# X1X1010/XequiNet

Measured on AMD Instinct MI355X. Metric: edges/sec + achieved HBM GB/s, energy+force inference, QM9-shape batch, higher is better.
Workload: dtype f32

## Files before the change

include/xeq.h:

```cpp
#ifndef XEQ_H
#define XEQ_H
#include <stdint.h>

#ifdef __cplusplus
extern "C" {
#endif

enum { XEQ_F32 = 0, XEQ_F64 = 1 };
enum { XEQ_RBF_BESSEL = 0, XEQ_RBF_GAUSSIAN = 1, XEQ_RBF_EXPBERN = 2, XEQ_RBF_EXPNORM = 3 };
enum { XEQ_CUTOFF_COSINE = 0, XEQ_CUTOFF_POLYNOMIAL = 1 };
enum {
  XEQ_OK = 0,
  XEQ_ERR_INVALID_ARGUMENT = 1,
  XEQ_ERR_LAUNCH = 2,
  XEQ_ERR_UNSUPPORTED = 3
};

int xeq_version(void);
const char* xeq_last_error(void);
int64_t xeq_launch_count(void);
int64_t xeq_launch_names(int64_t first, char* buf, int64_t cap);


int xeq_csr_rowptr(const int64_t* keys, int64_t n_keys, int64_t n_rows, int32_t* rowptr, void* stream);
// ... 317 lines not shown
int64_t xeq_rowptr_from_degrees_max(void);

int xeq_node_block_supported(int dtype, int node_dim, const int32_t mul[3]);
int xeq_node_block_auto(int64_t n);
int64_t xeq_small_rows_limit(void);
int xeq_node_block_set_waves(int waves);
int64_t xeq_node_block_rows(int64_t n);
int64_t xeq_node_block_fwd_tiles(int with_tail);
int xeq_node_block_pack_fwd(const float* w3, const float* uv0, const float* uv1, const float* uv2, const float* dot, const float* w4,
                            const float* w1_next, const float* w2_next, void* out, void* stream);
int xeq_node_block_fwd(int64_t n, const float* s, const float* x, const float* ln_w, const float* ln_b, const float* eq_w, const float* eq_b,
                       const float* b_uv, const float* b3, const float* b4, double eps, const void* packed, float* p_scratch, float* uv_bt, float* stats,
                       float* pre, float* a, float* ip, float* s_out, float* x_out, const float* ln_w_next, const float* ln_b_next,
                       const float* eq_w_next, const float* eq_b_next, const float* b1_next, const float* b2_next, float* stats_next,
                       float* xhat_next, float* pre_next, float* h_next, void* stream);
int64_t xeq_node_block_bwd_tiles(int with_tail, int with_gx);
int xeq_node_block_pack_bwd(const float* w3, const float* uv0, const float* uv1, const float* uv2, const float* dot, const float* w4,
                            const float* w1_next, const float* w2_next, int with_gx, void* out, void* stream);
int xeq_node_block_bwd(int64_t n, const float* g_h, const float* g_xhat_next, const float* g_s_in, const float* g_x_in, const float* s_out,
                       const float* x_out, const float* stats_next, const float* pre_next, const float* ln_w_next, const float* eq_w_next,
                       const float* uv_bt, const float* a, const float* ip, const float* pre, const float* s, const float* x,
                       const float* stats, const float* ln_w, const float* eq_w, double eps, const void* packed, float* gxo, float* gp,
                       float* gv, float* gw, float* g_s, float* g_x, void* stream);
int xeq_node_block_linear_test(const float* x, int64_t n, const float* w, int n_ot, int form, void* packed_scratch, float* y, void* stream);

#ifdef __cplusplus
}
#endif
#endif
```

xequinet_amd/csrc/xeq_nodeblock.hip:

```cpp
#include <stdlib.h>
#include <atomic>

#include <vector>

#include "xeq_common.h"

namespace xeq {
namespace nb {

typedef float tile_t __attribute__((ext_vector_type(8)));
typedef float f32x4 __attribute__((ext_vector_type(4)));
typedef float f32x8 __attribute__((ext_vector_type(8)));
typedef __bf16 bf16x8 __attribute__((ext_vector_type(8)));

constexpr int F = 128, M0 = 128, M1 = 64, M2 = 32, C = M0 + M1 + M2, D = M0 + 3 * M1 + 5 * M2;
constexpr int HM = F + 2 * C;
constexpr int AU = C + 2 * F;
constexpr int WAVE_ROWS = 16;
constexpr int ROWS_WG = 64;
constexpr int MAX_WAVES = 8;
constexpr int TILE_U4 = 192;
#ifndef XEQ_NB_STAGE
#define XEQ_NB_STAGE 4
#endif
// ... 541 lines not shown

struct FwdArgs {
  int64_t n;
  const float *s, *x;
  const float *lnw, *lnb, *eqw, *eqb;
  const float* b_uv;
  const float *b3, *b4;
  float eps;
  const uint4* wp;
  int n_tiles;
  float* p;
  float *uv, *stats, *pre, *a, *ip;
  float *s_out, *x_out;
  const float *lnw2, *lnb2, *eqw2, *eqb2, *b1n, *b2n;
  float *stats2, *xhat2, *pre2, *h2;
};

template <bool TAIL>
__global__ void __launch_bounds__(64 * MAX_WAVES, 1) k_node_block_fwd(FwdArgs a) {
  extern __shared__ uint4 ring[];
  const int lane = threadIdx.x & 63, wave = __builtin_amdgcn_readfirstlane(threadIdx.x >> 6);
  const int n = lane & 15, h = lane >> 4;
  const int n_waves = (int)(blockDim.x >> 6);
  const int64_t node = ((int64_t)blockIdx.x * n_waves + wave) * WAVE_ROWS + n;
  const bool ok = node < a.n;
  const int64_t row = ok ? node : a.n - 1;
  const int64_t N = a.n;
  NB_STAMP(0);
  NB_RSTAMP(17);
  WStream w;
  w.init(a.wp, ring, a.n_tiles, lane, wave & 3);
  const Park pk{ring + RING_BYTES / 16 + wave * PARK_U4 + lane};
  NB_STAMP(1);
// ... 208 lines not shown
      }
      st_xm<5>(xor_ + M0 + 3 * M1, h, X, ok);
    }
  }
  NB_STAMP(8);
  tile_t IP[4] = {zero16(), zero16(), zero16(), zero16()};
  {
    tile_t pt = ld_nat(pw, 0, lane);
    for (int t = 0; t < 7; ++t) {
      const tile_t cur = pt;
      if (t + 1 < 7) pt = ld_nat(pw, t + 1, lane);
      accum_tile<4>(w, IP, cur);
    }
  }
  tile_t SN[4];
  float* __restrict__ sor = a.s_out + row * F;
#pragma unroll
  for (int c = 0; c < 4; ++c) {
    const tile_t bsv = ld_par(a.b4, C + 32 * c, h), bss = ld_par(a.b4, C + F + 32 * c, h), S = ld_tile(srow, 32 * c, h);
    NB_SAVE(st_nat(ipw, c, lane, IP[c]));
    tile_t asv = zero16(), ass = zero16();
    out_pair_p<4>(w, asv, ass, pk);
    asv += bsv;
    ass += bss;
    NB_SAVE(st_nat(aw, 7 + c, lane, asv));
    NB_SAVE(st_nat(aw, 11 + c, lane, ass));
#pragma unroll
    for (int r = 0; r < 8; ++r) SN[c][r] = (S[r] + asv[r] * IP[c][r]) + ass[r];
    st_tile(sor, 32 * c, h, SN[c], ok);
  }
  NB_STAMP(9);
  if (!TAIL) return;

  const float mean_n = row_sum((sum16(SN[0]) + sum16(SN[1])) + (sum16(SN[2]) + sum16(SN[3]))) * (1.f / F);
  const float var_n = row_sum((sumsq16(SN[0], mean_n) + sumsq16(SN[1], mean_n)) + (sumsq16(SN[2], mean_n) + sumsq16(SN[3], mean_n))) * (1.f / F);
  const float rstd_n = 1.f / sqrtf(var_n + 1e-5f);
  const float mean0_n = row_sum(s0) * (1.f / M0);
  tile_t XN0[4];
#pragma unroll
  for (int t = 0; t < 4; ++t) XN0[t] = ld_tile(xor_, 32 * t, h);
  tile_t HN[4] = {zero16(), zero16(), zero16(), zero16()};
#pragma unroll
  for (int t = 0; t < 4; ++t) {
    const tile_t wv = ld_par(a.lnw2, 32 * t, h), bv = ld_par(a.lnb2, 32 * t, h);
    tile_t sh;
#pragma unroll
// ... 58 lines not shown
      }
    }
  }
  NB_STAMP(13);
  NB_RSTAMP(18);
#ifdef XEQ_NB_STAMPS
  if (lane == 0 && blockIdx.x < 1024) {
    g_nb_stamps[((int)blockIdx.x * 4 + wave) * NB_STAMPS + 14] = w.t_commit;
    g_nb_stamps[((int)blockIdx.x * 4 + wave) * NB_STAMPS + 15] = w.t_barrier;
    unsigned hw_, xcc_;
    asm volatile("s_getreg_b32 %0, hwreg(HW_REG_HW_ID)" : "=s"(hw_));
    asm volatile("s_getreg_b32 %0, hwreg(HW_REG_XCC_ID)" : "=s"(xcc_));
    g_nb_stamps[((int)blockIdx.x * 4 + wave) * NB_STAMPS + 16] = ((unsigned long long)xcc_ << 32) | hw_;
  }
#endif
}

enum { B_W2N = 0, B_W1N = 1, B_W4 = 2, B_W3 = 3, B_DOT = 4, B_UV0 = 5, B_UV1 = 6, B_UV2 = 7 };
static void program_bwd(bool tail, bool gx, std::vector<Seg>& p) {
  p.clear();
  if (tail) {
    p.push_back({B_W2N, 0, 4, 1, 0, HM / 32, 1, 0});
    p.push_back({B_W1N, 0, 4, 1, 0, 4, 1, 1});
  }
  if (gx) p.push_back({B_W4, 0, 4, 1, 0, 7, 1, 0});
  p.push_back({B_W4, 0, 4, 1, 7, 8, 1, 0});
  p.push_back({B_W3, 0, 4, 1, 0, 4, 1, 1});
  p.push_back({B_W3, 4, 7, 1, 0, 4, 1, 1});
  p.push_back({B_DOT, 0, 7, 1, 0, 4, 1, 1});
  for (int c = 0; c < 4; ++c) p.push_back({B_UV0, 0, 4, 1, c, 2, M0 / 32, 0});
// ... 454 lines not shown
    for (int m = 0; m < 5; ++m) {
      GW[m] = ld_nat(gww, x_tile(2, m, 0), lane);
      if (GX) R[m] = ld_nat(gxow, x_tile(2, m, 0), lane);
    }
#pragma unroll
    for (int m = 0; m < 5; ++m)
#pragma unroll
      for (int r = 0; r < 8; ++r) X[m][r] = (rr * GW[m][r] - coef * X[m][r]) + (GX ? R[m][r] : 0.f);
    st_xm<5>(gxr + M0 + 3 * M1, h, X, ok);
  }
}

static hipError_t raise_lds() {
  static hipError_t err = [] {
    const void* fns[] = {reinterpret_cast<const void*>(&k_node_block_fwd<true>), reinterpret_cast<const void*>(&k_node_block_fwd<false>),
                         reinterpret_cast<const void*>(&k_node_block_bwd<true, true>), reinterpret_cast<const void*>(&k_node_block_bwd<false, true>),
                         reinterpret_cast<const void*>(&k_node_block_bwd<false, false>)};
    hipError_t e = hipSuccess;
    for (const void* f : fns) {
      const hipError_t r = hipFuncSetAttribute(f, hipFuncAttributeMaxDynamicSharedMemorySize, lds_bytes(MAX_WAVES));
      if (r != hipSuccess) e = r;
    }
    return e;
  }();
  return err;
}

static std::atomic<int> g_waves_override{0};
static int waves_for(int64_t n) {
  const char* v = getenv("XEQ_NODE_BLOCK_WAVES");
// ... 77 lines not shown
                "xeq_node_block_fwd: null buffer");
  XEQ_CHECK_ARG(!tail || (x_out && ln_w_next && ln_b_next && eq_w_next && eq_b_next && b1_next && b2_next && stats_next && xhat_next && pre_next),
                "xeq_node_block_fwd: null buffer (next block)");
  FwdArgs fa;
  fa.n = n; fa.s = s; fa.x = x; fa.lnw = ln_w; fa.lnb = ln_b; fa.eqw = eq_w; fa.eqb = eq_b; fa.b_uv = b_uv; fa.b3 = b3; fa.b4 = b4;
  fa.eps = (float)eps; fa.wp = (const uint4*)packed; fa.n_tiles = (int)xeq_node_block_fwd_tiles(tail);
  fa.p = p_scratch; fa.uv = uv_bt; fa.stats = stats; fa.pre = pre; fa.a = a; fa.ip = ip; fa.s_out = s_out; fa.x_out = x_out;
  fa.lnw2 = ln_w_next; fa.lnb2 = ln_b_next; fa.eqw2 = eq_w_next; fa.eqb2 = eq_b_next; fa.b1n = b1_next; fa.b2n = b2_next;
  fa.stats2 = stats_next; fa.xhat2 = xhat_next; fa.pre2 = pre_next; fa.h2 = h_next;
  const int nw = waves_for(n);
  const dim3 grid((unsigned)((n + nw * WAVE_ROWS - 1) / (nw * WAVE_ROWS)));
  XEQ_CHECK_ARG(raise_lds() == hipSuccess, "xeq_node_block_fwd: cannot raise the dynamic LDS limit");
  if (tail) hipLaunchKernelGGL(k_node_block_fwd<true>, grid, dim3(64 * nw), lds_bytes(nw), (hipStream_t)stream, fa);
  else hipLaunchKernelGGL(k_node_block_fwd<false>, grid, dim3(64 * nw), lds_bytes(nw), (hipStream_t)stream, fa);
  XEQ_CHECK_LAUNCH("xeq_node_block_fwd");
  return XEQ_OK;
}

int64_t xeq_node_block_bwd_tiles(int with_tail, int with_gx) {
  std::vector<Seg> p;
  program_bwd(with_tail != 0, with_gx != 0 || with_tail != 0, p);
  return padded_tiles(seg_tiles(p));
}

int xeq_node_block_pack_bwd(const float* w3, const float* uv0, const float* uv1, const float* uv2, const float* dot, const float* w4,
                            const float* w1n, const float* w2n, int with_gx, void* out, void* stream) {
  XEQ_CHECK_ARG(w3 && uv0 && uv1 && uv2 && dot && w4 && out && ((w1n == nullptr) == (w2n == nullptr)), "xeq_node_block_pack_bwd: null buffer");
  const bool tail = w1n != nullptr;
  std::vector<Seg> p;
  program_bwd(tail, tail || with_gx != 0, p);
// ... 55 lines not shown
```

xequinet_amd/csrc/xeq_torch.cpp:

```cpp
#include <ATen/ATen.h>
#include <c10/hip/HIPStream.h>
#include <hip/hip_runtime_api.h>
#include <torch/csrc/autograd/custom_function.h>
#include <torch/library.h>

#include <cmath>
#include <cstdlib>
#include <mutex>
#include <optional>
#include <unordered_map>
#include <vector>

#include "../../include/xeq.h"

namespace {

using at::Tensor;
using torch::autograd::AutogradContext;
using torch::autograd::variable_list;

#define XCALL(...)                                                                                  \
  do {                                                                                              \
    const int st_ = (__VA_ARGS__);                                                                  \
    TORCH_CHECK(st_ == 0, "xequinet_amd: ", #__VA_ARGS__, " failed (", st_, "): ", xeq_last_error()); \
// ... 615 lines not shown
                            g.fwd.dbasis.defined() ? g.fwd.dbasis.data_ptr() : nullptr, st));
  } else {
    const int w = xeq_edge_basis_width(hy.B);
    g.sb_basis = at::empty({E, w}, fopt);
    g.sb_dbasis = at::empty({E, w}, fopt);
    XCALL(xeq_edge_basis(dt, vec.data_ptr(), E, hy.rbf_kind, hy.cutoff_kind, hy.B, hy.cutoff, p0.data_ptr(), OP(p1),
                         g.sb_basis.data_ptr(), g.sb_dbasis.data_ptr(), st));
  }

  auto wq_w = [&](const Tensor* q) {
    const Tensor* pk = wq_weight_pack(q[4], q[5], hy.B, F, mul);
    TORCH_CHECK(pk != nullptr, "xeq::xpainn_eval: rbf_lin weights cannot be packed for the wq kernels");
    return pk;
  };
  const bool nb_ok = dt == XEQ_F32 && hy.layer_norm && xeq_node_block_supported(XEQ_F32, F, mul) && xeq_node_block_auto(N);
  for (int b = 0; b < hy.blocks; ++b) {
    const Tensor* q = &prm[P_BLOCK0 + P_PER_BLOCK * b];
    {
      MsgSaved& m = msv[b];
      if (b > 0 && !m.h.defined()) {
        m.s = s;
        m.x = x;
        NormOut no = norm_fwd(hy, s, x, q[6], q[7], q[8], q[9], Tensor(), 0);
        m.stats = no.stats;
        m.xhat = no.xhat;
        mlp_fwd(no.shat, q[0], q[1], q[2], q[3], m.pre, m.h);
      }
      Tensor s_out = at::empty_like(s), x_out = at::empty_like(x);
      m.impl = impl;
      if (impl == 0) {
// ... 17 lines not shown
      u.s = s;
      u.x = x;
      const bool last_blk = b == hy.blocks - 1;
      if (nb_ok) {
        const Tensor* qn = last_blk ? nullptr : &prm[P_BLOCK0 + P_PER_BLOCK * (b + 1)];
        const NbPacks* pk = nb_packs(q, qn, !last_blk);
        auto fp = [](const Tensor& t) { return t.defined() ? (const float*)t.data_ptr() : nullptr; };
        auto fpm = [](Tensor& t) { return t.defined() ? (float*)t.data_ptr() : nullptr; };
        const int64_t NR = xeq_node_block_rows(N);
        u.uv = at::empty({2 * NR * D}, fopt);
        u.stats = at::empty({N, 4}, fopt);
        u.pre = at::empty({NR, F}, fopt);
        u.a = at::empty({NR, C + 2 * F}, fopt);
        u.ip = at::empty({NR, F}, fopt);
        Tensor p_scr = at::empty({NR, C}, fopt);
        Tensor s_out = at::empty_like(s), x_out = last_blk ? Tensor() : at::empty_like(x);
        MsgSaved* mn = last_blk ? nullptr : &msv[b + 1];
        if (mn) {
          mn->stats = at::empty({N, 4}, fopt);
          mn->xhat = at::empty({N * D}, fopt);
          mn->pre = at::empty({NR, F}, fopt);
          mn->h = at::empty({N, H}, fopt);
        }
        XCALL(xeq_node_block_fwd(N, fp(s), fp(x), fp(q[19]), fp(q[20]), fp(q[21]), fp(q[22]), fp(pk->bias_uv), fp(q[16]), fp(q[18]),
                                 hy.inv_eps, pk->fwd.data_ptr(), fpm(p_scr), fpm(u.uv), fpm(u.stats), fpm(u.pre), fpm(u.a), fpm(u.ip),
                                 fpm(s_out), fpm(x_out), qn ? fp(qn[6]) : nullptr, qn ? fp(qn[7]) : nullptr, qn ? fp(qn[8]) : nullptr,
                                 qn ? fp(qn[9]) : nullptr, qn ? fp(qn[1]) : nullptr, qn ? fp(qn[3]) : nullptr,
                                 mn ? fpm(mn->stats) : nullptr, mn ? fpm(mn->xhat) : nullptr, mn ? fpm(mn->pre) : nullptr,
                                 mn ? fpm(mn->h) : nullptr, st));
        s = s_out;
// ... 23 lines not shown
          const Tensor& W = q[10 + xb[k].l];
          if (xb[k].l == 0 && q[13].numel() > 0) at::addmm_out(ub[k].view, q[13], xb[k].view, W);
          else at::mm_out(ub[k].view, xb[k].view, W);
        }
        XCALL(xeq_uv_reduce_fwd(dt, u.uv.data_ptr(), N, mul, hy.inv_eps, cat.data_ptr(), F + C, F, p.data_ptr(), st));
      }
      mlp_and_linear_fwd(cat, q[15], q[16], q[17], q[18], p, q[14], u.pre, u.a, u.ip);
      const bool last = b == hy.blocks - 1;
      Tensor s_out = at::empty_like(s), x_out = last ? Tensor() : at::empty_like(x);
      XCALL(xeq_update_out_fwd(dt, s.data_ptr(), x.data_ptr(), u.uv.data_ptr(), u.a.data_ptr(), u.ip.data_ptr(), N, F, mul,
                               s_out.data_ptr(), last ? nullptr : x_out.data_ptr(), st));
      s = s_out;
      x = x_out;
    }
  }
  const Tensor* t = &prm[P_BLOCK0 + P_PER_BLOCK * hy.blocks];
  const LinPack* head_pk = dt == XEQ_F32 && t[0].size(0) % 4 == 0 && t[2].size(0) == 1 ? lin_pack(t[0], t[1]) : nullptr;
  const bool head_native = head_pk != nullptr && head_pk->bwd.defined();
  Tensor pre_o, atomic, jac;
  const bool head_fused = head_native && s.stride(1) == 1 && s.stride(0) % 4 == 0 && t[1].defined() && t[1].numel() > 0 &&
                          xeq_head_supported(XEQ_F32, F, (int)t[0].size(0));
  if (head_fused) {
    atomic = at::empty({N}, fopt);
    if (compute_forces || compute_virial) jac = at::empty({N, (int64_t)F}, fopt);
    XCALL(xeq_head_fwd(s.data_ptr(), s.stride(0), N, F, (int)t[0].size(0), head_pk->fwd.data_ptr(), head_pk->bwd.data_ptr(), t[2].data_ptr(),
                       t[3].data_ptr(), atomic.data_ptr(), jac.defined() ? jac.data_ptr() : nullptr, st));
  } else if (head_native) {
    const Tensor hidden = linear_fwd(s, t[0], t[1], 1, nullptr, &pre_o);
    atomic = at::empty({N}, fopt);
    XCALL(xeq_head_dot(hidden.data_ptr(), N, (int)t[0].size(0), t[2].data_ptr(), t[3].data_ptr(), atomic.data_ptr(), st));
  } else {
    pre_o = at::addmm(t[1], s, t[0].t());
    atomic = at::addmm(t[3], at::silu(pre_o), t[2].t()).reshape({-1});
  }
  Tensor energy = at::empty({G}, fopt);
  XCALL(xeq_segment_sum(dt, atomic.data_ptr(), (const int64_t*)ptr64.data_ptr(), G, 1, energy.data_ptr(), st));

// ... 339 lines not shown
```

xequinet_amd/lib.py:

```python
from __future__ import annotations

import ctypes
import os
from ctypes import c_char_p, c_double, c_int, c_int32, c_int64, c_void_p
from typing import Optional

import torch

_HERE = os.path.dirname(os.path.abspath(__file__))
LIB_PATH = os.environ.get("XEQ_LIB_PATH") or os.path.join(_HERE, "libxeq_hip.so")

XEQ_F32, XEQ_F64 = 0, 1
COPY_MANY_MAX = 16
SB_ACCUM_VEC = 16
XHAT_HIGHER_L_ZERO = 2
SB_Y0_ZERO = 8
SB_Q_ACCUMULATE = 16
SB_NO_GY = 32
WQ_MIRROR_WALK = 4
WQ_PACKED_WEIGHTS = 64
WQ_MAX_PART_SETS = 8
RBF_KINDS = {"bessel": 0, "gaussian": 1, "expbern": 2, "expnorm": 3}
CUTOFF_KINDS = {"cosine": 0, "polynomial": 1}

# ... 134 lines not shown
    "xeq_mlp2_fwd": [_P, c_int64, c_int64, c_int, _P, _P, c_int, _P, _P, c_int64, _P],
    "xeq_mlp2_bwd": [_P, c_int64, c_int64, c_int, _P, _P, _P, c_int, _P, c_int64, _P],
    "xeq_mlp2_and_linear": [c_int, _P, c_int64, c_int64, c_int, _P, _P, c_int, _P, _P, c_int64, _P, c_int64, c_int, _P, c_int, _P, c_int64, _P],
    "xeq_pack_epoch": [],
    "xeq_pack_epoch_bump": [],
    "xeq_rowptr_guard": [_P, c_int64, c_int64, _P, _P, _P],
    "xeq_node_block_supported": [c_int, c_int, _I3],
    "xeq_node_block_fwd_tiles": [c_int],
    "xeq_node_block_rows": [c_int64],
    "xeq_node_block_auto": [c_int64],
    "xeq_small_rows_limit": [],
    "xeq_node_block_set_waves": [c_int],
    "xeq_node_block_pack_fwd": [_P, _P, _P, _P, _P, _P, _P, _P, _P, _P],
    "xeq_node_block_fwd": [c_int64, _P, _P, _P, _P, _P, _P, _P, _P, _P, c_double, _P, _P, _P, _P, _P, _P, _P, _P, _P, _P, _P, _P, _P, _P, _P,
                           _P, _P, _P, _P, _P],
    "xeq_node_block_linear_test": [_P, c_int64, _P, c_int, c_int, _P, _P, _P],
    "xeq_node_block_bwd_tiles": [c_int, c_int],
    "xeq_node_block_pack_bwd": [_P, _P, _P, _P, _P, _P, _P, _P, c_int, _P, _P],
    "xeq_node_block_bwd": [c_int64, _P, _P, _P, _P, _P, _P, _P, _P, _P, _P, _P, _P, _P, _P, _P, _P, _P, _P, _P, c_double, _P, _P, _P, _P, _P,
                           _P, _P, _P],
}
_RET_I64 = {"xeq_launch_count", "xeq_launch_names", "xeq_message_wq_packed_weight_floats", "xeq_rowptr_from_degrees_max", "xeq_csr_by_key_workspace", "xeq_message_wq_pcap", "xeq_message_wq_plan_workspace", "xeq_message_wq_win_ints",
            "xeq_message_wq_parts_floats", "xeq_mlp_packed_floats", "xeq_exclusive_scan_i32_workspace", "xeq_node_block_fwd_tiles", "xeq_node_block_bwd_tiles", "xeq_node_block_rows", "xeq_pack_epoch", "xeq_tensor_product_wgrad_chunks", "xeq_small_rows_limit"}
EXPORTS = ["xeq_version", "xeq_last_error", *_PROTOS]

_lib: Optional[ctypes.CDLL] = None


def load() -> ctypes.CDLL:
    global _lib
# ... 81 lines not shown
```

xequinet_amd/nn/fused.py:

```python
from __future__ import annotations

import math
from typing import Tuple

import torch
import torch.nn.functional as F_
from torch.autograd import Function
from torch.autograd.function import once_differentiable

from .. import lib, ops
from ..lib import call, dtype_code, mul3, ptr, stream

def _bt_blocks(buf: torch.Tensor, n: int, mul, width: int):
    out = []
    base = 0
    for l, m in enumerate(mul):
        d = 2 * l + 1
        if m > 0:
            out.append((l, m, buf[n * base * width : n * (base + d * m) * width].view(n * d, width * m)))
        base += d * m
    return out


def _norm_fwd(s, x, norm, o3norm, node_dim, mul, shat_out=None, ld=None):
# ... 316 lines not shown
    @staticmethod
    @once_differentiable
    def backward(ctx, g_atomic, g_total):
        if not ctx.saved_tensors or (g_atomic is None and g_total is None):
            return None, None, None, None
        jac, batch = ctx.saved_tensors
        n, F = jac.shape
        if g_atomic is not None and g_atomic.stride(0) not in (0, 1):
            g_atomic = g_atomic.contiguous()
        if g_total is not None and g_total.stride(0) not in (0, 1):
            g_total = g_total.contiguous()
        g_s = torch.empty_like(jac)
        call("xeq_head_bwd", ptr(jac), n, F, ptr(g_atomic), 0 if g_atomic is None else g_atomic.stride(0), ptr(g_total),
             0 if g_total is None else g_total.stride(0), ptr(batch), ptr(g_s), stream())
        return g_s, None, None, None


class EmbeddingLinear(Function):

    @staticmethod
    def forward(ctx, z32, table, lin, weight, bias):
        out = _linear(table, _linear_pack(lin, weight, bias, False), weight.shape[1], weight.shape[0], bias is not None, row_index=z32)[0]
        ctx.save_for_backward(z32, table)
        ctx.has_bias = bias is not None
        return out

    @staticmethod
    @once_differentiable
    def backward(ctx, g):
        z32, table = ctx.saved_tensors
# ... 289 lines not shown
```

xequinet_amd/nn/model.py:

```python
from __future__ import annotations

from typing import Dict, Iterable, List, Optional, Union

import torch
import torch.nn as nn

from . import training
from .basic import compute_edge_data, compute_properties
from .output import resolve_output
from .xpainn import XEmbedding, XPainnMessage, XPainnUpdate

_E3NN_ONLY = (".rsh_conv.", ".tp.", ".scalar_mul.", ".sph_harm.", ".output_mask", "._", ".invariant.tp", ".equidot.tp")


class BaseModel(nn.Module):
    cutoff_radius: float

    def __init__(self) -> None:
        super().__init__()
        self.mods = nn.ModuleDict()
        self.extra_properties = []
        self.native_training = True

    def forward(
# ... 76 lines not shown
            )
        if action_blocks > 0:
            self.mods["embedding"]._next_message = [self.mods["message_0"]]
        for i in range(action_blocks - 1):
            self.mods[f"update_{i}"]._next_message = [self.mods[f"message_{i + 1}"]]
        if output_modes is None:
            output_modes = ["energy"]
        elif isinstance(output_modes, str) or not isinstance(output_modes, Iterable):
            output_modes = [output_modes]
        for mode in output_modes:
            output = resolve_output(mode, **kwargs)
            self.mods[f"output_{mode}"] = output
            self.extra_properties.extend(output.extra_properties)
        if action_blocks > 0 and all(not getattr(self.mods[f"output_{m}"], "reads_equivariant", False) for m in output_modes):
            self.mods[f"update_{action_blocks - 1}"].equivariant_output_unused = True


def resolve_model(model_name: str, **kwargs) -> BaseModel:
    models_factory = {"xpainn": XPaiNN}
    if model_name.lower() not in models_factory:
        raise NotImplementedError(f"Unsupported model {model_name}")
    return models_factory[model_name.lower()](**kwargs)


def load_model(ckpt_file: str, device: Optional[torch.device] = None):
    from ..data import NeighborTransform

    class ModelWithTransform:
        def __init__(self, model, transform, device):
            self.model = model
# ... 17 lines not shown
```

xequinet_amd/nn/nodeblock.py:

```python
from __future__ import annotations

from typing import Optional

import torch

from .. import lib
from ..lib import call, mul3, ptr, stream

TILE_BYTES = 3072
pack_epoch = lib.pack_epoch


def supported(update, message=None) -> bool:
    from .fused import _packed_uv

    if not isinstance(update.update_mlp[1], torch.nn.SiLU) or isinstance(update.norm, torch.nn.Identity):
        return False
    w = update.update_mlp[0].weight
    if w.dtype != torch.float32 or not w.is_cuda:
        return False
    if not lib.load().xeq_node_block_supported(lib.XEQ_F32, update.node_dim, mul3(update.node_irreps.mul3())):
        return False
    if update.update_mlp[0].bias is None or update.update_mlp[2].bias is None or update.dot_lin.bias is not None:
        return False
# ... 67 lines not shown
    if tail:
        o.update(stats2=torch.empty((n, 4), **f32), xhat2=torch.empty(n * D, **f32), pre2=torch.empty((rows, F), **f32),
                 h2=torch.empty((n, F + 2 * C), **f32))
    m = update.update_mlp
    nm = message
    call("xeq_node_block_fwd", n, ptr(s), ptr(x), ptr(update.norm.weight), ptr(update.norm.bias), ptr(update.o3norm.affine_weight),
         ptr(update.o3norm.affine_bias), ptr(_uv_bias(update)), ptr(m[0].bias), ptr(m[2].bias), float(update.invariant.eps), ptr(packed),
         ptr(o["p"]), ptr(o["uv"]), ptr(o["stats"]), ptr(o["pre"]), ptr(o["a"]), ptr(o["ip"]), ptr(o["s_out"]), ptr(o["x_out"]),
         ptr(nm.norm.weight if tail else None), ptr(nm.norm.bias if tail else None), ptr(nm.o3norm.affine_weight if tail else None),
         ptr(nm.o3norm.affine_bias if tail else None), ptr(nm.scalar_mlp[0].bias if tail else None),
         ptr(nm.scalar_mlp[2].bias if tail else None), ptr(o.get("stats2")), ptr(o.get("xhat2")), ptr(o.get("pre2")), ptr(o.get("h2")),
         stream())
    return o


def packed_bwd(update, message=None, with_gx: bool = True) -> torch.Tensor:
    from .fused import _packed_uv

    m = update.update_mlp
    ws = [m[0].weight, update.update_U.weight, update.update_V.weight, update.dot_lin.weight, m[2].weight]
    if message is not None:
        ws += [message.scalar_mlp[0].weight, message.scalar_mlp[2].weight]
    with_gx = bool(with_gx or message is not None)
    key = (_versions(*ws), pack_epoch(), id(message), with_gx)
    cache = getattr(update, "_xeq_nb_bwd", None)
    if cache is None:
        cache = update._xeq_nb_bwd = {}
    hit = cache.get(with_gx)
    if hit is not None and hit[0] == key:
        return hit[1]
# ... 41 lines not shown
```

xequinet_amd/nn/output.py:

```python
from __future__ import annotations

from typing import Dict, List

import torch
import torch.nn as nn

from .. import keys
from ..scatter import scatter_sum
from . import training
from .basic import resolve_activation


class OutputModule(nn.Module):
    extra_properties: List[str]

    def __init__(self) -> None:
        super().__init__()

    def forward(self, data: Dict[str, torch.Tensor]) -> Dict[str, torch.Tensor]:
        raise NotImplementedError


class EnergyOut(OutputModule):
    def __init__(
# ... 7 lines not shown
    ) -> None:
        super().__init__()
        self.node_dim = node_dim
        self.hidden_dim = hidden_dim
        final_linear = nn.Linear(self.hidden_dim, 1)
        final_linear.weight.data *= node_scale
        nn.init.constant_(final_linear.bias, node_shift)
        self.out_mlp = nn.Sequential(
            nn.Linear(self.node_dim, self.hidden_dim),
            resolve_activation(activation),
            final_linear,
        )
        self.extra_properties = [keys.TOTAL_ENERGY, keys.ATOMIC_ENERGIES]

    def forward(self, data: Dict[str, torch.Tensor]) -> Dict[str, torch.Tensor]:
        if training.active(self, data):
            return training.energy_out(self, data)
        batch = data[keys.BATCH]
        node_scalar = data[keys.NODE_INVARIANT]
        from .fused import EnergyHead, EnergyReadout

        ptr_ = data.get(keys.BATCH_PTR)
        if (ptr_ is not None and keys.ATOMIC_ENERGIES not in data and not data.get(training.PARAM_GRADS, False)
                and EnergyReadout.supported(self.out_mlp, node_scalar)):
            atomic_energies, total_energy = EnergyReadout.apply(node_scalar, self.out_mlp, batch.to(torch.int64).contiguous(), ptr_)
            data[keys.ATOMIC_ENERGIES] = atomic_energies
            data[keys.TOTAL_ENERGY] = total_energy
            return data
        if EnergyHead.supported(self.out_mlp, node_scalar):
            params = EnergyHead.params(self.out_mlp) if data.get(training.PARAM_GRADS, False) else ()
# ... 18 lines not shown
```

xequinet_amd/nn/xpainn.py:

```python
from __future__ import annotations

from typing import Dict, Iterable, Optional

import torch
import torch.nn as nn

from .. import keys, o3, ops
from .basic import Int2c1eEmbedding, edge_graph, resolve_activation
from . import training
from . import nodeblock
from .fused import EmbeddingLinear, MessageBlock, NodeBlock, UpdateBlock, message_params, update_params
from .o3layer import EquivariantDot, EquivariantLayerNorm, Invariant
from .rbf import resolve_cutoff, resolve_rbf

RADIAL_SPEC = "_xeq_radial_spec"
EQUIVARIANT_IS_ZERO = "_xeq_equivariant_is_zero"
ZERO_EQUIVARIANT = "_xeq_zero_equivariant"
PRESTAGE = "_xeq_message_prestage"
FIRST_FRONT = "_xeq_first_front"
ELEMENT_ROWS = "_xeq_element_rows"


class XEmbedding(nn.Module):

    def __init__(
        self,
# ... 201 lines not shown
        self.update_V = o3.Linear(self.node_irreps, self.node_irreps, biases=True)
        self.invariant = Invariant(self.node_irreps)
        self.equidot = EquivariantDot(self.node_irreps)
        self.dot_lin = nn.Linear(self.node_num_irreps, self.node_dim, bias=False)
        self.rsh_conv = o3.ElementwiseTensorProduct(self.node_irreps, f"{self.node_num_irreps}x0e")
        self.update_mlp = nn.Sequential(
            nn.Linear(self.node_dim + self.node_num_irreps, self.node_dim),
            resolve_activation(activation),
            nn.Linear(self.node_dim, self.hidden_dim),
        )
        self.norm = nn.LayerNorm(self.node_dim) if layer_norm else nn.Identity()
        self.o3norm = EquivariantLayerNorm(self.node_irreps) if layer_norm else nn.Identity()
        self.fused = True
        self.equivariant_output_unused = False
        self._next_message = []

    def _node_block_ok(self, data) -> bool:
        s = data[keys.NODE_INVARIANT]
        return (s.is_cuda and s.dtype == torch.float32 and not data.get(training.PARAM_GRADS, False) and nodeblock.supported(self)
                and bool(ops.lib.load().xeq_node_block_auto(s.shape[0])))

    def forward(self, data: Dict[str, torch.Tensor]) -> Dict[str, torch.Tensor]:
        if training.active(self, data):
            return training.update(self, data)
        if self.fused and self._node_block_ok(data):
            nxt = self._next_message[0] if self._next_message else None
            if nxt is not None and not (nxt.fused and nodeblock.supported(self, nxt)):
                nxt = None
            out = NodeBlock.apply(data[keys.NODE_INVARIANT], data[keys.NODE_EQUIVARIANT], self, nxt)
            data[keys.NODE_INVARIANT], data[keys.NODE_EQUIVARIANT] = out[0], out[1]
            if nxt is not None:
                data[PRESTAGE] = out
            return data
        if self.fused:
            params = update_params(self) if data.get(training.PARAM_GRADS, False) else ()
            s_new, x_new = UpdateBlock.apply(data[keys.NODE_INVARIANT], data[keys.NODE_EQUIVARIANT], self, *params)
            data[keys.NODE_INVARIANT] = s_new
            data[keys.NODE_EQUIVARIANT] = x_new
            return data
        node_scalar = self.norm(data[keys.NODE_INVARIANT])
        node_equi = self.o3norm(data[keys.NODE_EQUIVARIANT])

        U_equi = self.update_U(node_equi)
# ... 18 lines not shown
```

Measured before the change: 180.6 million.

## Fuse energy readout head into last node-block forward kernel

Measured after the change: 184.0 million, median of 6. 1.02x the previous value.

```diff
diff --git a/include/xeq.h b/include/xeq.h
--- a/include/xeq.h
+++ b/include/xeq.h
@@ -355,6 +355,11 @@
                        float* pre, float* a, float* ip, float* s_out, float* x_out, const float* ln_w_next, const float* ln_b_next,
                        const float* eq_w_next, const float* eq_b_next, const float* b1_next, const float* b2_next, float* stats_next,
                        float* xhat_next, float* pre_next, float* h_next, void* stream);
+int xeq_node_block_head_supported(int node_dim, int hidden_dim);
+int xeq_node_block_fwd_head(int64_t n, const float* s, const float* x, const float* ln_w, const float* ln_b, const float* eq_w, const float* eq_b,
+                            const float* b_uv, const float* b3, const float* b4, double eps, const void* packed, float* p_scratch, float* uv_bt,
+                            float* stats, float* pre, float* a, float* ip, float* s_out, int hidden_dim, const void* w1_packed,
+                            const void* w1t_packed, const float* w2, const float* b2, float* atomic, float* jac, void* stream);
 int64_t xeq_node_block_bwd_tiles(int with_tail, int with_gx);
 int xeq_node_block_pack_bwd(const float* w3, const float* uv0, const float* uv1, const float* uv2, const float* dot, const float* w4,
                             const float* w1_next, const float* w2_next, int with_gx, void* out, void* stream);
diff --git a/xequinet_amd/csrc/xeq_nodeblock.hip b/xequinet_amd/csrc/xeq_nodeblock.hip
--- a/xequinet_amd/csrc/xeq_nodeblock.hip
+++ b/xequinet_amd/csrc/xeq_nodeblock.hip
@@ -579,9 +579,15 @@
   float *s_out, *x_out;
   const float *lnw2, *lnb2, *eqw2, *eqb2, *b1n, *b2n;
   float *stats2, *xhat2, *pre2, *h2;
+  int hH;
+  const float *hw1p, *hw1tp, *hw2, *hb2;
+  float *atomic, *jac;
 };
 
-template <bool TAIL>
+constexpr int HEAD_XLD = F + 4, HEAD_HMAX = 64, HEAD_HLD = HEAD_HMAX + 4;
+__device__ __forceinline__ void head_rows(const FwdArgs& a, const tile_t (&SN)[4], float* __restrict__ hs, int lane, int64_t row, bool ok);
+
+template <bool TAIL, bool HEAD = false>
 __global__ void __launch_bounds__(64 * MAX_WAVES, 1) k_node_block_fwd(FwdArgs a) {
   extern __shared__ uint4 ring[];
   const int lane = threadIdx.x & 63, wave = __builtin_amdgcn_readfirstlane(threadIdx.x >> 6);
@@ -820,7 +826,7 @@
     }
   }
   tile_t SN[4];
-  float* __restrict__ sor = a.s_out + row * F;
+  float* __restrict__ sor = (HEAD && !a.s_out) ? nullptr : a.s_out + row * F;
 #pragma unroll
   for (int c = 0; c < 4; ++c) {
     const tile_t bsv = ld_par(a.b4, C + 32 * c, h), bss = ld_par(a.b4, C + F + 32 * c, h), S = ld_tile(srow, 32 * c, h);
@@ -833,9 +839,13 @@
     NB_SAVE(st_nat(aw, 11 + c, lane, ass));
 #pragma unroll
     for (int r = 0; r < 8; ++r) SN[c][r] = (S[r] + asv[r] * IP[c][r]) + ass[r];
-    st_tile(sor, 32 * c, h, SN[c], ok);
+    if (!HEAD || sor) st_tile(sor, 32 * c, h, SN[c], ok);
   }
   NB_STAMP(9);
+  if (HEAD) {
+    asm volatile("" ::: "memory");
+    head_rows(a, SN, reinterpret_cast<float*>(ring + RING_BYTES / 16 + wave * PARK_U4), lane, row, ok);
+  }
   if (!TAIL) return;
 
   const float mean_n = row_sum((sum16(SN[0]) + sum16(SN[1])) + (sum16(SN[2]) + sum16(SN[3]))) * (1.f / F);
@@ -924,6 +934,110 @@
     g_nb_stamps[((int)blockIdx.x * 4 + wave) * NB_STAMPS + 16] = ((unsigned long long)xcc_ << 32) | hw_;
   }
 #endif
+}
+
+__device__ __forceinline__ void head_rows(const FwdArgs& a, const tile_t (&SN)[4], float* __restrict__ hs, int lane, int64_t row, bool ok) {
+  const int i = lane & 15, kq = lane >> 4, kh = kq & 1;
+  const bool sel = (kq >> 1) != 0;
+  const int H = a.hH;
+  constexpr int G = F / 8;
+#pragma unroll
+  for (int c = 0; c < 4; ++c)
+#pragma unroll
+    for (int g = 0; g < 2; ++g)
+      *reinterpret_cast<float4*>(hs + i * HEAD_XLD + 32 * c + 16 * g + 4 * kq) = make_float4(SN[c][4 * g], SN[c][4 * g + 1], SN[c][4 * g + 2], SN[c][4 * g + 3]);
+  const float* xs = hs + i * HEAD_XLD + 4 * kh;
+  auto ld_w1 = [&](int t, float (&wa)[G][2], float& bias_a) {
+    const float4* wp = reinterpret_cast<const float4*>(a.hw1p) + (int64_t)(t >> 1) * (G + 1) * 64 + 16 * (t & 1) + i + 32 * kh;
+#pragma unroll
+    for (int q = 0; q < G; ++q) {
+      const float4 v = wp[q * 64];
+      wa[q][0] = sel ? v.y : v.x;
+      wa[q][1] = sel ? v.w : v.z;
+    }
+    bias_a = kq == 0 ? reinterpret_cast<const float*>(wp + G * 64)[0] : 0.f;
+  };
+  f32x4 pre[HEAD_HMAX / 16];
+  float wa[2][G][2], ba[2];
+  ld_w1(0, wa[0], ba[0]);
+#pragma unroll
+  for (int t = 0; t < HEAD_HMAX / 16; ++t) {
+    if (16 * t >= H) break;
+    if (16 * (t + 1) < H && t + 1 < HEAD_HMAX / 16) ld_w1(t + 1, wa[(t + 1) & 1], ba[(t + 1) & 1]);
+    const int b = t & 1;
+    f32x4 h0 = {0.f, 0.f, 0.f, 0.f}, h1 = {0.f, 0.f, 0.f, 0.f};
+#pragma unroll
+    for (int q = 0; q < G / 2; ++q) {
+      const float4 xv = *reinterpret_cast<const float4*>(xs + 8 * q);
+      h0 = __builtin_amdgcn_mfma_f32_16x16x4f32(wa[b][q][0], sel ? xv.y : xv.x, h0, 0, 0, 0);
+      h0 = __builtin_amdgcn_mfma_f32_16x16x4f32(wa[b][q][1], sel ? xv.w : xv.z, h0, 0, 0, 0);
+    }
+    h0 = __builtin_amdgcn_mfma_f32_16x16x4f32(ba[b], kq == 0 ? 1.f : 0.f, h0, 0, 0, 0);
+#pragma unroll
+    for (int q = G / 2; q < G; ++q) {
+      const float4 xv = *reinterpret_cast<const float4*>(xs + 8 * q);
+      h1 = __builtin_amdgcn_mfma_f32_16x16x4f32(wa[b][q][0], sel ? xv.y : xv.x, h1, 0, 0, 0);
+      h1 = __builtin_amdgcn_mfma_f32_16x16x4f32(wa[b][q][1], sel ? xv.w : xv.z, h1, 0, 0, 0);
+    }
+    pre[t] = h0 + h1;
+  }
+  const int GJ = H >> 3;
+  auto ld_w1t = [&](int t, float (&wj)[HEAD_HMAX / 8][2]) {
+    const float4* wp = reinterpret_cast<const float4*>(a.hw1tp) + (int64_t)(t >> 1) * (GJ + 1) * 64 + 16 * (t & 1) + i + 32 * kh;
+#pragma unroll
+    for (int q = 0; q < HEAD_HMAX / 8; ++q) {
+      const float4 v = wp[(q < GJ ? q : GJ - 1) * 64];
+      wj[q][0] = sel ? v.y : v.x;
+      wj[q][1] = sel ? v.w : v.z;
+    }
+  };
+  float wj[2][HEAD_HMAX / 8][2];
+  if (a.jac) ld_w1t(0, wj[0]);
+  asm volatile("" ::: "memory");
+  float* Es = hs;
+  float* Gs = hs + 16 * HEAD_HLD;
+#pragma unroll
+  for (int t = 0; t < HEAD_HMAX / 16; ++t) {
+    if (16 * t >= H) break;
+    const int col = 16 * t + 4 * kq;
+    const float4 wv = *reinterpret_cast<const float4*>(a.hw2 + col);
+    const float wq4[4] = {wv.x, wv.y, wv.z, wv.w};
+    float e[4], gh[4];
+#pragma unroll
+    for (int c = 0; c < 4; ++c) {
+      const float x = pre[t][c];
+      const float sig = 1.f / (1.f + expf(-x));
+      e[c] = (x * sig) * wq4[c];
+      gh[c] = wq4[c] * (sig * (1.f + x * (1.f - sig)));
+    }
+    *reinterpret_cast<float4*>(&Es[i * HEAD_HLD + col]) = make_float4(e[0], e[1], e[2], e[3]);
+    *reinterpret_cast<float4*>(&Gs[i * HEAD_HLD + col]) = make_float4(gh[0], gh[1], gh[2], gh[3]);
+  }
+  {
+    float p0 = 0.f, p1 = 0.f;
+    for (int c = kq; c < H; c += 8) p0 += Es[i * HEAD_HLD + c];
+    for (int c = kq + 4; c < H; c += 8) p1 += Es[i * HEAD_HLD + c];
+    float acc = p0 + p1;
+    acc += __shfl_xor(acc, 32, 64);
+    acc += __shfl_xor(acc, 16, 64);
+    if (ok && kq == 0) a.atomic[row] = acc + (a.hb2 ? a.hb2[0] : 0.f);
+  }
+  if (!a.jac) return;
+  const float* gs = Gs + i * HEAD_HLD + 4 * kh;
+#pragma unroll
+  for (int t = 0; t < F / 16; ++t) {
+    if (t + 1 < F / 16) ld_w1t(t + 1, wj[(t + 1) & 1]);
+    const int b = t & 1;
+    f32x4 acc = {0.f, 0.f, 0.f, 0.f};
+#pragma unroll
+    for (int q = 0; q < HEAD_HMAX / 8; ++q)
+      if (q < GJ) {
+        const float4 gv = *reinterpret_cast<const float4*>(gs + 8 * q);
+        acc = __builtin_amdgcn_mfma_f32_16x16x4f32(wj[b][q][0], sel ? gv.y : gv.x, acc, 0, 0, 0);
+        acc = __builtin_amdgcn_mfma_f32_16x16x4f32(wj[b][q][1], sel ? gv.w : gv.z, acc, 0, 0, 0);
+      }
+    if (ok) *reinterpret_cast<float4*>(a.jac + row * F + 16 * t + 4 * kq) = make_float4(acc[0], acc[1], acc[2], acc[3]);
+  }
 }
 
 enum { B_W2N = 0, B_W1N = 1, B_W4 = 2, B_W3 = 3, B_DOT = 4, B_UV0 = 5, B_UV1 = 6, B_UV2 = 7 };
@@ -1408,6 +1522,7 @@
 static hipError_t raise_lds() {
   static hipError_t err = [] {
     const void* fns[] = {reinterpret_cast<const void*>(&k_node_block_fwd<true>), reinterpret_cast<const void*>(&k_node_block_fwd<false>),
+                         reinterpret_cast<const void*>(&k_node_block_fwd<false, true>),
                          reinterpret_cast<const void*>(&k_node_block_bwd<true, true>), reinterpret_cast<const void*>(&k_node_block_bwd<false, true>),
                          reinterpret_cast<const void*>(&k_node_block_bwd<false, false>)};
     hipError_t e = hipSuccess;
@@ -1515,6 +1630,33 @@
   if (tail) hipLaunchKernelGGL(k_node_block_fwd<true>, grid, dim3(64 * nw), lds_bytes(nw), (hipStream_t)stream, fa);
   else hipLaunchKernelGGL(k_node_block_fwd<false>, grid, dim3(64 * nw), lds_bytes(nw), (hipStream_t)stream, fa);
   XEQ_CHECK_LAUNCH("xeq_node_block_fwd");
+  return XEQ_OK;
+}
+
+int xeq_node_block_head_supported(int node_dim, int hidden_dim) {
+  return node_dim == F && (hidden_dim == 32 || hidden_dim == HEAD_HMAX) && xeq_head_supported(XEQ_F32, node_dim, hidden_dim);
+}
+
+int xeq_node_block_fwd_head(int64_t n, const float* s, const float* x, const float* ln_w, const float* ln_b, const float* eq_w, const float* eq_b,
+                            const float* b_uv, const float* b3, const float* b4, double eps, const void* packed, float* p_scratch, float* uv_bt,
+                            float* stats, float* pre, float* a, float* ip, float* s_out, int hidden_dim, const void* w1_packed,
+                            const void* w1t_packed, const float* w2, const float* b2, float* atomic, float* jac, void* stream) {
+  XEQ_CHECK_ARG(n >= 0 && n < ((int64_t)1 << 31) / (2 * D), "xeq_node_block_fwd_head: n = %lld out of range", (long long)n);
+  XEQ_CHECK_ARG(xeq_node_block_head_supported(F, hidden_dim), "xeq_node_block_fwd_head: hidden width %d (32 or 64)", hidden_dim);
+  if (n == 0) return XEQ_OK;
+  XEQ_CHECK_ARG(s && x && ln_w && ln_b && eq_w && eq_b && b3 && b4 && packed && p_scratch && uv_bt && stats && pre && a && ip && w1_packed &&
+                w2 && atomic && (w1t_packed || !jac), "xeq_node_block_fwd_head: null buffer");
+  FwdArgs fa{};
+  fa.n = n; fa.s = s; fa.x = x; fa.lnw = ln_w; fa.lnb = ln_b; fa.eqw = eq_w; fa.eqb = eq_b; fa.b_uv = b_uv; fa.b3 = b3; fa.b4 = b4;
+  fa.eps = (float)eps; fa.wp = (const uint4*)packed; fa.n_tiles = (int)xeq_node_block_fwd_tiles(0);
+  fa.p = p_scratch; fa.uv = uv_bt; fa.stats = stats; fa.pre = pre; fa.a = a; fa.ip = ip; fa.s_out = s_out; fa.x_out = nullptr;
+  fa.hH = hidden_dim; fa.hw1p = (const float*)w1_packed; fa.hw1tp = (const float*)w1t_packed; fa.hw2 = w2; fa.hb2 = b2;
+  fa.atomic = atomic; fa.jac = jac;
+  const int nw = waves_for(n);
+  const dim3 grid((unsigned)((n + nw * WAVE_ROWS - 1) / (nw * WAVE_ROWS)));
+  XEQ_CHECK_ARG(raise_lds() == hipSuccess, "xeq_node_block_fwd_head: cannot raise the dynamic LDS limit");
+  hipLaunchKernelGGL((k_node_block_fwd<false, true>), grid, dim3(64 * nw), lds_bytes(nw), (hipStream_t)stream, fa);
+  XEQ_CHECK_LAUNCH("xeq_node_block_fwd_head");
   return XEQ_OK;
 }
 
diff --git a/xequinet_amd/csrc/xeq_torch.cpp b/xequinet_amd/csrc/xeq_torch.cpp
--- a/xequinet_amd/csrc/xeq_torch.cpp
+++ b/xequinet_amd/csrc/xeq_torch.cpp
@@ -653,6 +653,12 @@
     return pk;
   };
   const bool nb_ok = dt == XEQ_F32 && hy.layer_norm && xeq_node_block_supported(XEQ_F32, F, mul) && xeq_node_block_auto(N);
+  const Tensor* t = &prm[P_BLOCK0 + P_PER_BLOCK * hy.blocks];
+  const LinPack* head_pk = dt == XEQ_F32 && t[0].size(0) % 4 == 0 && t[2].size(0) == 1 ? lin_pack(t[0], t[1]) : nullptr;
+  const bool head_native = head_pk != nullptr && head_pk->bwd.defined();
+  const bool head_in_nb = nb_ok && head_native && t[1].defined() && t[1].numel() > 0 && xeq_head_supported(XEQ_F32, F, (int)t[0].size(0)) &&
+                          xeq_node_block_head_supported(F, (int)t[0].size(0));
+  Tensor pre_o, atomic, jac;
   for (int b = 0; b < hy.blocks; ++b) {
     const Tensor* q = &prm[P_BLOCK0 + P_PER_BLOCK * b];
     {
@@ -700,6 +706,17 @@
         u.a = at::empty({NR, C + 2 * F}, fopt);
         u.ip = at::empty({NR, F}, fopt);
         Tensor p_scr = at::empty({NR, C}, fopt);
+        if (last_blk && head_in_nb) {
+          atomic = at::empty({N}, fopt);
+          if (compute_forces || compute_virial) jac = at::empty({N, (int64_t)F}, fopt);
+          XCALL(xeq_node_block_fwd_head(N, fp(s), fp(x), fp(q[19]), fp(q[20]), fp(q[21]), fp(q[22]), fp(pk->bias_uv), fp(q[16]), fp(q[18]),
+                                        hy.inv_eps, pk->fwd.data_ptr(), fpm(p_scr), fpm(u.uv), fpm(u.stats), fpm(u.pre), fpm(u.a),
+                                        fpm(u.ip), nullptr, (int)t[0].size(0), head_pk->fwd.data_ptr(), head_pk->bwd.data_ptr(),
+                                        fp(t[2]), fp(t[3]), fpm(atomic), fpm(jac), st));
+          s = Tensor();
+          x = Tensor();
+          continue;
+        }
         Tensor s_out = at::empty_like(s), x_out = last_blk ? Tensor() : at::empty_like(x);
         MsgSaved* mn = last_blk ? nullptr : &msv[b + 1];
         if (mn) {
@@ -753,13 +770,10 @@
       x = x_out;
     }
   }
-  const Tensor* t = &prm[P_BLOCK0 + P_PER_BLOCK * hy.blocks];
-  const LinPack* head_pk = dt == XEQ_F32 && t[0].size(0) % 4 == 0 && t[2].size(0) == 1 ? lin_pack(t[0], t[1]) : nullptr;
-  const bool head_native = head_pk != nullptr && head_pk->bwd.defined();
-  Tensor pre_o, atomic, jac;
-  const bool head_fused = head_native && s.stride(1) == 1 && s.stride(0) % 4 == 0 && t[1].defined() && t[1].numel() > 0 &&
-                          xeq_head_supported(XEQ_F32, F, (int)t[0].size(0));
-  if (head_fused) {
+  const bool head_fused = head_in_nb || (head_native && s.stride(1) == 1 && s.stride(0) % 4 == 0 && t[1].defined() && t[1].numel() > 0 &&
+                                         xeq_head_supported(XEQ_F32, F, (int)t[0].size(0)));
+  if (head_in_nb) {
+  } else if (head_fused) {
     atomic = at::empty({N}, fopt);
     if (compute_forces || compute_virial) jac = at::empty({N, (int64_t)F}, fopt);
     XCALL(xeq_head_fwd(s.data_ptr(), s.stride(0), N, F, (int)t[0].size(0), head_pk->fwd.data_ptr(), head_pk->bwd.data_ptr(), t[2].data_ptr(),
diff --git a/xequinet_amd/lib.py b/xequinet_amd/lib.py
--- a/xequinet_amd/lib.py
+++ b/xequinet_amd/lib.py
@@ -172,6 +172,9 @@
     "xeq_node_block_pack_fwd": [_P, _P, _P, _P, _P, _P, _P, _P, _P, _P],
     "xeq_node_block_fwd": [c_int64, _P, _P, _P, _P, _P, _P, _P, _P, _P, c_double, _P, _P, _P, _P, _P, _P, _P, _P, _P, _P, _P, _P, _P, _P, _P,
                            _P, _P, _P, _P, _P],
+    "xeq_node_block_head_supported": [c_int, c_int],
+    "xeq_node_block_fwd_head": [c_int64, _P, _P, _P, _P, _P, _P, _P, _P, _P, c_double, _P, _P, _P, _P, _P, _P, _P, _P, c_int, _P, _P, _P, _P,
+                                _P, _P, _P],
     "xeq_node_block_linear_test": [_P, c_int64, _P, c_int, c_int, _P, _P, _P],
     "xeq_node_block_bwd_tiles": [c_int, c_int],
     "xeq_node_block_pack_bwd": [_P, _P, _P, _P, _P, _P, _P, _P, c_int, _P, _P],
diff --git a/xequinet_amd/nn/fused.py b/xequinet_amd/nn/fused.py
--- a/xequinet_amd/nn/fused.py
+++ b/xequinet_amd/nn/fused.py
@@ -354,6 +354,55 @@
         call("xeq_head_bwd", ptr(jac), n, F, ptr(g_atomic), 0 if g_atomic is None else g_atomic.stride(0), ptr(g_total),
              0 if g_total is None else g_total.stride(0), ptr(batch), ptr(g_s), stream())
         return g_s, None, None, None
+
+
+HEAD_DONE = "_xeq_head_done"
+
+
+class NodeBlockReadout(Function):
+
+    @staticmethod
+    def supported(update, seq: torch.nn.Sequential, s: torch.Tensor) -> bool:
+        from . import nodeblock
+
+        return EnergyReadout.supported(seq, s) and nodeblock.head_supported(update, seq)
+
+    @staticmethod
+    def forward(ctx, s, x, update, seq, batch, ptr_):
+        from . import nodeblock
+
+        s, x = s.contiguous(), x.contiguous()
+        want_bwd = ctx.needs_input_grad[0] or ctx.needs_input_grad[1]
+        o = nodeblock.node_block_fwd_head(s, x, update, seq, want_jac=want_bwd)
+        atomic = o["atomic"]
+        ptr64 = ptr_.to(torch.int64).contiguous()
+        total = torch.empty(ptr64.numel() - 1, dtype=s.dtype, device=s.device)
+        call("xeq_segment_sum", dtype_code(s), ptr(atomic), ptr(ptr64), ptr64.numel() - 1, 1, ptr(total), stream())
+        ctx.update = update
+        ctx.keys = ["uv", "stats", "pre", "a", "ip"]
+        ctx.save_for_backward(*((s, x, o["jac"], batch, *[o[k] for k in ctx.keys]) if want_bwd else ()))
+        ctx.set_materialize_grads(False)
+        return atomic, total
+
+    @staticmethod
+    @once_differentiable
+    def backward(ctx, g_atomic, g_total):
+        from . import nodeblock
+
+        if not ctx.saved_tensors or (g_atomic is None and g_total is None):
+            return None, None, None, None, None, None
+        s, x, jac, batch = ctx.saved_tensors[:4]
+        saved = dict(zip(ctx.keys, ctx.saved_tensors[4:]))
+        n, F = jac.shape
+        if g_atomic is not None and g_atomic.stride(0) not in (0, 1):
+            g_atomic = g_atomic.contiguous()
+        if g_total is not None and g_total.stride(0) not in (0, 1):
+            g_total = g_total.contiguous()
+        g_s_out = torch.empty_like(jac)
+        call("xeq_head_bwd", ptr(jac), n, F, ptr(g_atomic), 0 if g_atomic is None else g_atomic.stride(0), ptr(g_total),
+             0 if g_total is None else g_total.stride(0), ptr(batch), ptr(g_s_out), stream())
+        g_s, g_x = nodeblock.node_block_bwd(saved, s, x, ctx.update, None, g_s_out, None)
+        return g_s, g_x, None, None, None, None
 
 
 class EmbeddingLinear(Function):
diff --git a/xequinet_amd/nn/model.py b/xequinet_amd/nn/model.py
--- a/xequinet_amd/nn/model.py
+++ b/xequinet_amd/nn/model.py
@@ -114,6 +114,8 @@
             self.extra_properties.extend(output.extra_properties)
         if action_blocks > 0 and all(not getattr(self.mods[f"output_{m}"], "reads_equivariant", False) for m in output_modes):
             self.mods[f"update_{action_blocks - 1}"].equivariant_output_unused = True
+        if action_blocks > 0 and list(output_modes) == ["energy"]:
+            self.mods[f"update_{action_blocks - 1}"]._head = [self.mods["output_energy"]]
 
 
 def resolve_model(model_name: str, **kwargs) -> BaseModel:
diff --git a/xequinet_amd/nn/nodeblock.py b/xequinet_amd/nn/nodeblock.py
--- a/xequinet_amd/nn/nodeblock.py
+++ b/xequinet_amd/nn/nodeblock.py
@@ -105,6 +105,34 @@
     return o
 
 
+def head_supported(update, seq) -> bool:
+    return bool(lib.load().xeq_node_block_head_supported(update.node_dim, seq[0].weight.shape[0]))
+
+
+def node_block_fwd_head(s: torch.Tensor, x: torch.Tensor, update, seq, want_jac: bool) -> dict:
+    from .fused import _linear_pack
+
+    lib.require_hip(s, x)
+    n, D = x.shape
+    F = update.node_dim
+    C = update.node_irreps.num_irreps
+    f32 = dict(dtype=torch.float32, device=s.device)
+    packed = packed_fwd(update, None)
+    rows = int(lib.load().xeq_node_block_rows(n))
+    o = {"p": torch.empty((rows, C), **f32), "uv": torch.empty(2 * rows * D, **f32), "stats": torch.empty((n, 4), **f32),
+         "pre": torch.empty((rows, F), **f32), "a": torch.empty((rows, C + 2 * F), **f32), "ip": torch.empty((rows, F), **f32),
+         "atomic": torch.empty(n, **f32), "jac": torch.empty((n, F), **f32) if want_jac else None}
+    lin1, lin2 = seq[0], seq[2]
+    w2 = lin2.weight.detach().reshape(-1).contiguous()
+    m = update.update_mlp
+    call("xeq_node_block_fwd_head", n, ptr(s), ptr(x), ptr(update.norm.weight), ptr(update.norm.bias), ptr(update.o3norm.affine_weight),
+         ptr(update.o3norm.affine_bias), ptr(_uv_bias(update)), ptr(m[0].bias), ptr(m[2].bias), float(update.invariant.eps), ptr(packed),
+         ptr(o["p"]), ptr(o["uv"]), ptr(o["stats"]), ptr(o["pre"]), ptr(o["a"]), ptr(o["ip"]), None, lin1.weight.shape[0],
+         ptr(_linear_pack(lin1, lin1.weight, lin1.bias, False)), ptr(_linear_pack(lin1, lin1.weight, None, True) if want_jac else None),
+         ptr(w2), ptr(lin2.bias), ptr(o["atomic"]), ptr(o["jac"]), stream())
+    return o
+
+
 def packed_bwd(update, message=None, with_gx: bool = True) -> torch.Tensor:
     from .fused import _packed_uv
 
diff --git a/xequinet_amd/nn/output.py b/xequinet_amd/nn/output.py
--- a/xequinet_amd/nn/output.py
+++ b/xequinet_amd/nn/output.py
@@ -45,6 +45,10 @@
         self.extra_properties = [keys.TOTAL_ENERGY, keys.ATOMIC_ENERGIES]
 
     def forward(self, data: Dict[str, torch.Tensor]) -> Dict[str, torch.Tensor]:
+        from .fused import HEAD_DONE
+
+        if data.pop(HEAD_DONE, False):
+            return data
         if training.active(self, data):
             return training.energy_out(self, data)
         batch = data[keys.BATCH]
diff --git a/xequinet_amd/nn/xpainn.py b/xequinet_amd/nn/xpainn.py
--- a/xequinet_amd/nn/xpainn.py
+++ b/xequinet_amd/nn/xpainn.py
@@ -9,7 +9,7 @@
 from .basic import Int2c1eEmbedding, edge_graph, resolve_activation
 from . import training
 from . import nodeblock
-from .fused import EmbeddingLinear, MessageBlock, NodeBlock, UpdateBlock, message_params, update_params
+from .fused import HEAD_DONE, EmbeddingLinear, MessageBlock, NodeBlock, NodeBlockReadout, UpdateBlock, message_params, update_params
 from .o3layer import EquivariantDot, EquivariantLayerNorm, Invariant
 from .rbf import resolve_cutoff, resolve_rbf
 
@@ -241,6 +241,7 @@
         self.fused = True
         self.equivariant_output_unused = False
         self._next_message = []
+        self._head = []
 
     def _node_block_ok(self, data) -> bool:
         s = data[keys.NODE_INVARIANT]
@@ -254,6 +255,16 @@
             nxt = self._next_message[0] if self._next_message else None
             if nxt is not None and not (nxt.fused and nodeblock.supported(self, nxt)):
                 nxt = None
+            head = self._head[0].out_mlp if self._head else None
+            ptr_ = data.get(keys.BATCH_PTR)
+            if (nxt is None and head is not None and ptr_ is not None and getattr(self, "equivariant_output_unused", False)
+                    and keys.ATOMIC_ENERGIES not in data and NodeBlockReadout.supported(self, head, data[keys.NODE_INVARIANT])):
+                atomic, total = NodeBlockReadout.apply(data[keys.NODE_INVARIANT], data[keys.NODE_EQUIVARIANT], self, head,
+                                                       data[keys.BATCH].to(torch.int64).contiguous(), ptr_)
+                data[keys.NODE_INVARIANT], data[keys.NODE_EQUIVARIANT] = None, None
+                data[keys.ATOMIC_ENERGIES], data[keys.TOTAL_ENERGY] = atomic, total
+                data[HEAD_DONE] = True
+                return data
             out = NodeBlock.apply(data[keys.NODE_INVARIANT], data[keys.NODE_EQUIVARIANT], self, nxt)
             data[keys.NODE_INVARIANT], data[keys.NODE_EQUIVARIANT] = out[0], out[1]
             if nxt is not None:
```
